# wcy199705/DfFintheWild

Hardware: AMD Instinct MI355X
Metric: focal-stacks/sec (10x3x256x256) (higher is better)
Workload: dtype bf16x3 (split-bf16 MFMA operands hi+lo, fp32 accumulate, fp32-accurate); 1 GPU; DFF_net forward, 10-slice 3x256x256 focal stacks, batch 32 per GPU (BASELINE.json config 3), dense focus_dists, synthetic weights seed 0; batch_per_gpu=32, global_batch=32, slices=10, height=256, width=256, parallelism=single GPU, precision=bf16x3, input=float32 (B,3,N,H,W), the reference's tensor contract

## Files before the change

dffinthewild_amd/csrc/dffw_engine.cpp:

```cpp
#include <algorithm>
#include <cmath>
#include <cstdarg>
#include <cstdio>
#include <cstdlib>
#include <cstring>
#include <functional>
#include <map>
#include <memory>
#include <string>
#include <vector>

#include "dffw_run.h"
#include "dffw_srd_roll.h"
#include "dffw_stem.h"

namespace dffw {

static thread_local std::string g_err;
static thread_local std::string g_last_kernel;
static thread_local std::string g_last_op_kernels;
}
int dffw_fail(int code, const char *fmt, ...) {
    char buf[1024];
    va_list ap;
// ... 1012 lines not shown
}

int dffw_op_efd(int device, int precision, const float *x, int B, int Cin, int N, int H, int W, const float *ws, const float *bns,
                const float *wp, const float *bnp, int pooled_at_hand, float *y, void *hip_stream) {
    g_last_op_kernels.clear();
    if (!x || !ws || !bns || !wp || !bnp || !y) return fail(DFFW_EINVAL, "null argument");
    if (precision < 0 || precision > 2) return fail(DFFW_EINVAL, "unknown precision %d", precision);
    if (Cin != 8 && Cin != 16) return fail(DFFW_EINVAL, "the EFD blocks have 8 or 16 input channels, got %d", Cin);
    if (B < 1 || N < 1 || H < 2 || W < 2 || H % 2 || W % 2) return fail(DFFW_EINVAL, "bad shape (H and W must be even)");
    HIPCHK(hipSetDevice(device));
    const std::string p = Cin == 8 ? "DFF_net.FM_conv1.0" : "DFF_net.FM_conv2.0";
    const int Cout = 2 * Cin;
    Table t;
    t.efd(p, Cin, Cout);
    dffw_engine eng;
    eng.device = device;
    eng.prec = precision;
    const float *const wts[2] = {ws, wp}, *const bnv[2] = {bns, bnp};
    for (int i = 0; i < 2; ++i) {
        const int rc = pack_conv(t.layers[i], precision, wts[i], bnv[i], nullptr, eng.convs[t.layers[i].conv]);
        if (rc) return rc;
    }
    return run_block_op(eng, (hipStream_t)hip_stream, [&](Run &r) {
        Act in = r.act(B, N, H, W, Cin);
        if (r.ok() && !r.dry) r.check(launch_from_ncdhw(precision, x, in.p, B, Cin, N, H, W, r.s), "from_ncdhw");
        Act m;
        if (pooled_at_hand) m = r.pool(in, 0, 2);
        Act out = efd(r, p, in, &m);
        if (r.ok() && !r.dry) r.check(launch_to_ncdhw(precision, out.p, y, B, Cout, N, H / 2, W / 2, r.s), "to_ncdhw");
    });
}

int dffw_op_of_block(int device, int precision, const float *x, int B, int Cin, int N, int H, int W, int Cout, int stride,
                     const float *w0, const float *bn0, const float *w2, const float *bn2, const float *wf, float *y, void *hip_stream) {
    g_last_op_kernels.clear();
    if (!x || !w0 || !bn0 || !w2 || !bn2 || !wf || !y) return fail(DFFW_EINVAL, "null argument");
    if (precision < 0 || precision > 2) return fail(DFFW_EINVAL, "unknown precision %d", precision);
    static const struct { int cin, cout, s; const char *name; } blocks[] = {
        {3, 8, 1, "OF_feature.0"}, {8, 8, 1, "OF_feature.1"}, {8, 16, 2, "OF_feature1.0"},
        {16, 16, 1, "OF_feature1.1"}, {16, 32, 2, "OF_feature2.0"}, {32, 32, 1, "OF_feature2.1"}};
    const char *name = nullptr;
    for (const auto &b : blocks)
        if (b.cin == Cin && b.cout == Cout && b.s == stride) name = b.name;
    if (!name) return fail(DFFW_EINVAL, "no alignment feature block has (Cin, Cout, stride) = (%d, %d, %d)", Cin, Cout, stride);
    if (B < 1 || N < 1 || H < 1 || W < 1 || H % stride || W % stride) return fail(DFFW_EINVAL, "bad shape (H and W must be multiples of the stride)");
    HIPCHK(hipSetDevice(device));
    const std::string p = std::string("optical_flow_aggregation.") + name;
    Table t;
    t.of_block(p, Cin, Cout, stride);
    dffw_engine eng;
    eng.device = device;
    eng.prec = precision;
    for (const LayerDef &L : t.layers) {
        if (L.folded) continue;
        const bool sc = !L.shortcut.empty();
        const float *w = L.conv == p + ".conv.0.0" ? w0 : L.conv == p + ".conv.2.0" ? w2 : wf;
        const float *bn = L.conv == p + ".conv.0.0" ? bn0 : L.conv == p + ".conv.2.0" ? bn2 : nullptr;
        const int rc = pack_conv(L, precision, w, bn, nullptr, eng.convs[L.conv], sc ? wf : nullptr, sc ? Cin : 0);
        if (rc) return rc;
    }
    return run_block_op(eng, (hipStream_t)hip_stream, [&](Run &r) {
        Act out;
        if (Cin == 3) {
            out = of_first_block(r, p, x, B, N, H, W);
        } else {
            Act in = r.act(B, N, H, W, Cin);
            if (r.ok() && !r.dry) r.check(launch_from_ncdhw(precision, x, in.p, B, Cin, N, H, W, r.s), "from_ncdhw");
            out = of_block(r, p, in);
        }
        if (r.ok() && !r.dry) r.check(launch_to_ncdhw(precision, out.p, y, B, Cout, N, H / stride, W / stride, r.s), "to_ncdhw");
    });
}

int dffw_op_regress(int device, const float *score, int B, int N, int h, int w, int H, int W, const float *focus_dists,
                    const int64_t fd_strides[4], float *depth, void *hip_stream) {
    if (!score || !focus_dists || !fd_strides || !depth) return fail(DFFW_EINVAL, "null argument");
    HIPCHK(hipSetDevice(device));
    hipStream_t s = (hipStream_t)hip_stream;
    HIPCHK(launch_regress(score, B, N, h, w, H, W, focus_dists, fd_strides[0], fd_strides[1], fd_strides[2], fd_strides[3], depth, s));
    HIPCHK(hipStreamSynchronize(s));
    return DFFW_OK;
}

int dffw_op_fov_warp(int device, const float *x, int B, int C, int N, int H, int W, const float *alpha, const float *fovs,
                     int alpha_from_sample0, float *out, float *flow, void *hip_stream) {
    if (!x || !alpha || !fovs || !out) return fail(DFFW_EINVAL, "null argument");
    if (B < 1 || C < 1 || N < 1 || H < 1 || W < 1) return fail(DFFW_EINVAL, "bad shape");
    HIPCHK(hipSetDevice(device));
    hipStream_t s = (hipStream_t)hip_stream;
    HIPCHK(launch_fov_warp(x, alpha, fovs, out, flow, B, C, N, H, W, alpha_from_sample0, s));
    HIPCHK(hipStreamSynchronize(s));
    return DFFW_OK;
}

}
```

dffinthewild_amd/csrc/dffw_kernels.hip:

```cpp
#include <cstdio>
#include <cstdlib>

#include "dffw_device.h"
#include "dffw_internal.h"
#include "dffw_persist.h"

namespace dffw {

template <int PREC, int NT, int MT>
__global__ __launch_bounds__(256) void conv_igemm(const ConvArgs a) {
    constexpr int PARTS = Fmt<PREC>::PARTS;
    constexpr bool F16 = (PREC == P_FP16);
    const int lane = threadIdx.x & 63;
    const int wave = threadIdx.x >> 6;
    const int g = lane >> 4, r = lane & 15;
    const int64_t pos0 = ((int64_t)blockIdx.x * 4 + wave) * (MT * 16);
    if (pos0 >= a.M) return;

    const int ps0 = PARTS * a.C0, ps1 = PARTS * a.C1;
    const int64_t samp0 = (int64_t)a.Ni * a.Hi * a.Wi * ps0;
    const int64_t samp1 = (int64_t)a.Ni * a.Hi * a.Wi * ps1;

    int pn[MT], py[MT], px[MT], pbase[MT];
    bool pv[MT];
// ... 1083 lines not shown
                    const float v = hy * (hx * s00[k] + lx * s01[k]) + ly * (hx * s10[k] + lx * s11[k]);
                    const float p = softplus_fast(v) + 1e-6f;
                    den += p;
                    num += f[k] * p;
                }
            }
        }
        depth[i] = num / den;
    }
}

template <int NMAX>
__global__ __launch_bounds__(256) void regress_fused_kernel(const RegressHeads hd, int B, int N, int H, int W, const float *__restrict__ fd, int64_t fsb,
                                                            int64_t fsn, int64_t fsh, int64_t fsw) {
    const unsigned total = (unsigned)B * H * W;
    for (unsigned u = blockIdx.x * blockDim.x + threadIdx.x; u < total; u += gridDim.x * blockDim.x) {
        const unsigned t = u / (unsigned)W;
        const int X = (int)(u - t * (unsigned)W);
        const unsigned bb = t / (unsigned)H;
        const int Y = (int)(t - bb * (unsigned)H);
        const float *fp = fd + bb * fsb + Y * fsh + X * fsw;
        float f[NMAX];
#pragma unroll
        for (int n = 0; n < NMAX; ++n) f[n] = fp[(n < N ? n : N - 1) * fsn];
        for (int head = 0; head < hd.n; ++head) {
            const float *__restrict__ score = hd.score[head];
            const int h = hd.h[head], w = hd.w[head];
            const float *sp = score + (int64_t)bb * N * h * w;
            float num = 0.f, den = 0.f;
            if (h == H && w == W) {
                const int o = Y * w + X;
                float sv[NMAX];
#pragma unroll
                for (int n = 0; n < NMAX; ++n) sv[n] = sp[(int64_t)(n < N ? n : N - 1) * h * w + o];
#pragma unroll
                for (int n = 0; n < NMAX; ++n) {
                    if (n < N) {
                        const float p = softplus_fast(sv[n]) + 1e-6f;
                        den += p;
                        num += f[n] * p;
                    }
                }
            } else {
                const float sch = (float)h / (float)H, scw = (float)w / (float)W;
                float sy = ((float)Y + 0.5f) * sch - 0.5f;
                float sx = ((float)X + 0.5f) * scw - 0.5f;
                sy = sy < 0.f ? 0.f : sy;
                sx = sx < 0.f ? 0.f : sx;
                const int y0 = (int)sy, x0 = (int)sx;
                const int y1 = y0 + (y0 < h - 1 ? 1 : 0), x1 = x0 + (x0 < w - 1 ? 1 : 0);
                const float ly = sy - (float)y0, lx = sx - (float)x0;
                const float hy = 1.f - ly, hx = 1.f - lx;
                const int o00 = y0 * w + x0, o01 = y0 * w + x1, o10 = y1 * w + x0, o11 = y1 * w + x1;
#pragma unroll
                for (int n0 = 0; n0 < NMAX; n0 += 5) {
                    if (n0 < N) {
                        float s00[5], s01[5], s10[5], s11[5];
#pragma unroll
                        for (int k = 0; k < 5; ++k) {
                            const int n = n0 + k < N ? n0 + k : N - 1;
                            const float *pl = sp + (int64_t)n * h * w;
                            s00[k] = pl[o00];
                            s01[k] = pl[o01];
                            s10[k] = pl[o10];
                            s11[k] = pl[o11];
                        }
#pragma unroll
                        for (int k = 0; k < 5; ++k) {
                            if (n0 + k < N) {
                                const float v = hy * (hx * s00[k] + lx * s01[k]) + ly * (hx * s10[k] + lx * s11[k]);
                                const float p = softplus_fast(v) + 1e-6f;
                                den += p;
                                num += f[n0 + k < NMAX ? n0 + k : NMAX - 1] * p;
                            }
                        }
                    }
                }
            }
            hd.depth[head][u] = num / den;
        }
    }
}

hipError_t launch_regress_heads(const RegressHeads &hd, int B, int N, int H, int W, const float *fd, int64_t fsb, int64_t fsn, int64_t fsh,
                                int64_t fsw, hipStream_t s) {
    if (hd.n < 1 || hd.n > 4) return hipErrorInvalidValue;
    const int64_t total = (int64_t)B * H * W;
    if (hd.n > 1 && N <= 16 && total < (1ll << 31) && !hd.nofuse) {
        if (N <= 10) hipLaunchKernelGGL((regress_fused_kernel<10>), dim3(grid_for(total)), dim3(256), 0, s, hd, B, N, H, W, fd, fsb, fsn, fsh, fsw);
        else hipLaunchKernelGGL((regress_fused_kernel<16>), dim3(grid_for(total)), dim3(256), 0, s, hd, B, N, H, W, fd, fsb, fsn, fsh, fsw);
        return hipGetLastError();
    }
    hipLaunchKernelGGL(regress_kernel, dim3(grid_for(total), (unsigned)hd.n), dim3(256), 0, s, hd, B, N, H, W, fd, fsb, fsn, fsh, fsw);
    return hipGetLastError();
}

hipError_t launch_regress(const float *score, int B, int N, int h, int w, int H, int W, const float *fd, int64_t fsb,
                          int64_t fsn, int64_t fsh, int64_t fsw, float *depth, hipStream_t s) {
    RegressHeads hd{};
    hd.n = 1;
    hd.score[0] = score;
    hd.depth[0] = depth;
    hd.h[0] = h;
    hd.w[0] = w;
    return launch_regress_heads(hd, B, N, H, W, fd, fsb, fsn, fsh, fsw, s);
}

__global__ void set_raw_kernel(RawStack rs, RawStack *dst) { *dst = rs; }
hipError_t launch_set_raw(const RawStack &rs, RawStack *dst, hipStream_t s) {
    hipLaunchKernelGGL(set_raw_kernel, dim3(1), dim3(1), 0, s, rs, dst);
    return hipGetLastError();
}

}
```

dffinthewild_amd/engine.py:

```python
import ctypes
import os
import threading
from ctypes import POINTER, byref, c_char_p, c_float, c_int, c_int64, c_void_p

import torch

_HERE = os.path.dirname(os.path.abspath(__file__))
LIB_PATH = os.environ.get("DFFW_LIB_PATH") or os.path.join(_HERE, "libdffw.so")

PRECISIONS = {"bf16x3": 0, "fp16": 1, "bf16": 2}
NET_DEPTH = 0
NET_E2E = 1


class DffwError(RuntimeError):
    pass


class _Tensor(ctypes.Structure):
    _fields_ = [("name", c_char_p), ("data", POINTER(c_float)), ("numel", c_int64)]


class _Tap(ctypes.Structure):
    _fields_ = [("name", c_char_p), ("dst", c_void_p), ("numel", c_int64)]


class _Prof(ctypes.Structure):
    _fields_ = [("kernel", c_char_p), ("layer", c_char_p), ("flops", ctypes.c_double), ("bytes", ctypes.c_double),
                ("ms", c_float)]


class SimParams(ctypes.Structure):
    _fields_ = [("pixel_per_meter", ctypes.c_double), ("min_depth", ctypes.c_double), ("max_depth", ctypes.c_double),
                ("min_focus", ctypes.c_double), ("max_focus", ctypes.c_double), ("num_planes", c_int), ("max_radius", c_int)]


def _load():
    if not os.path.exists(LIB_PATH):
        raise DffwError(
            f"{LIB_PATH} not found: build the HIP extension first "
            "(python -c 'import __graft_entry__ as g; g.build()' or make -C dffinthewild_amd/csrc). "
            "dffinthewild_amd has no CPU fallback.")
    lib = ctypes.CDLL(LIB_PATH)
    lib.dffw_version.restype = c_char_p
    lib.dffw_last_error.restype = c_char_p
    lib.dffw_last_conv_kernel.restype = c_char_p
    lib.dffw_param_count.argtypes = [c_int]
    lib.dffw_param_info.argtypes = [c_int, c_int, POINTER(c_char_p), POINTER(c_int64), POINTER(c_int), POINTER(c_int)]
    lib.dffw_engine_create.argtypes = [c_int, c_int, POINTER(_Tensor), c_int, c_int, POINTER(c_void_p)]
    lib.dffw_engine_destroy.argtypes = [c_void_p]
    lib.dffw_engine_destroy.restype = None
    lib.dffw_engine_precision.argtypes = [c_void_p]
    lib.dffw_workspace_bytes.argtypes = [c_void_p, c_int, c_int, c_int, c_int]
    lib.dffw_workspace_bytes.restype = c_int64
    fwd = [c_void_p, c_void_p, c_void_p, POINTER(c_int64), c_int, c_int, c_int, c_int,
           POINTER(c_void_p), c_void_p, c_int64, c_void_p]
    lib.dffw_forward.argtypes = fwd
    lib.dffw_forward_taps.argtypes = fwd + [POINTER(_Tap), c_int]
    lib.dffw_forward_e2e.argtypes = [c_void_p, c_void_p, c_void_p, POINTER(c_int64), c_void_p, c_int, c_int, c_int, c_int,
                                     POINTER(c_void_p), c_void_p, c_void_p, c_int64, c_void_p, POINTER(_Tap), c_int]
    lib.dffw_forward_raw.argtypes = [c_void_p, c_void_p, c_int, POINTER(c_int64), c_int, c_int, c_void_p, POINTER(c_int64), c_int, c_int, c_int,
                                     c_int, POINTER(c_void_p), c_void_p, c_int64, c_void_p]
    lib.dffw_profile_enable.argtypes = [c_void_p, c_int]
    lib.dffw_profile_collect.argtypes = [c_void_p, POINTER(_Prof), c_int]
    lib.dffw_op_conv3d.argtypes = [c_int, c_int, c_void_p, c_int, c_int, c_int, c_int, c_int, POINTER(c_float), c_int,
                                   POINTER(c_int), POINTER(c_int), POINTER(c_int), POINTER(c_int), c_int,
                                   POINTER(c_float), POINTER(c_float), c_void_p, c_int, c_void_p, c_void_p]
    lib.dffw_op_conv3d_ex.argtypes = [c_int, c_int, c_void_p, c_int, c_int, c_int, c_int, c_int, POINTER(c_float), c_int,
                                      POINTER(c_int), POINTER(c_int), POINTER(c_int), POINTER(c_int), c_int,
                                      POINTER(c_float), POINTER(c_float), c_void_p, c_int, c_void_p, c_void_p, POINTER(c_float), c_void_p, c_void_p]
    lib.dffw_op_pool.argtypes = [c_int, c_int, c_int, c_int, c_void_p, c_int, c_int, c_int, c_int, c_int, c_void_p, c_void_p]
    lib.dffw_op_srd.argtypes = [c_int, c_int, c_void_p, c_int, c_int, c_int, c_int, c_int] + [POINTER(c_float)] * 6 + [c_void_p] * 3
    lib.dffw_op_efd.argtypes = [c_int, c_int, c_void_p, c_int, c_int, c_int, c_int, c_int] + [POINTER(c_float)] * 4 + [c_int, c_void_p, c_void_p]
    lib.dffw_op_of_block.argtypes = [c_int, c_int, c_void_p] + [c_int] * 7 + [POINTER(c_float)] * 5 + [c_void_p] * 2
    lib.dffw_last_op_kernels.restype = c_char_p
    lib.dffw_op_fov_warp.argtypes = [c_int, c_void_p, c_int, c_int, c_int, c_int, c_int, c_void_p, c_void_p, c_int,
                                     c_void_p, c_void_p, c_void_p]
    lib.dffw_op_regress.argtypes = [c_int, c_void_p, c_int, c_int, c_int, c_int, c_int, c_int, c_void_p,
                                    POINTER(c_int64), c_void_p, c_void_p]
    c_u8p = POINTER(ctypes.c_uint8)
    lib.dffw_pack_stack.argtypes = [c_int, c_void_p, c_int, POINTER(c_int64), c_int, c_int, c_int, c_int, c_int, c_int, c_void_p, c_void_p]
    lib.dffw_augment_stack.argtypes = [c_int, c_void_p, c_int, POINTER(c_int64)] + [c_int] * 6 + [c_void_p, c_int] + [c_void_p] * 6 + \
                                      [c_int, c_float, c_float, c_float, c_void_p]
    lib.dffw_unpack_stack.argtypes = [c_int, c_void_p, c_int, c_int, c_int, c_int, c_int, c_int, c_void_p, c_void_p]
    lib.dffw_colorize.argtypes = [c_int, c_void_p, c_int, c_int, c_int, c_int, c_int, c_int, c_float, c_float, c_void_p, c_void_p, c_void_p]
    lib.dffw_jet_lut.argtypes = [c_u8p]
    lib.dffw_metrics_scratch_bytes.argtypes = [c_int]
    lib.dffw_metrics_scratch_bytes.restype = c_int64
    lib.dffw_metrics.argtypes = [c_int, c_void_p, c_int, c_int, c_int, c_void_p, c_void_p, c_void_p, c_int, c_int, c_void_p, c_void_p,
                                 c_int64, c_void_p]
    lib.dffw_comm_unique_id.argtypes = [ctypes.c_char_p]
    lib.dffw_comm_init_rank.argtypes = [c_int, c_int, c_int, ctypes.c_char_p, POINTER(c_void_p)]
    lib.dffw_comm_init_all.argtypes = [c_int, POINTER(c_int), POINTER(c_void_p)]
    lib.dffw_comm_destroy.argtypes = [c_void_p]
    lib.dffw_comm_destroy.restype = None
    lib.dffw_comm_rank.argtypes = [c_void_p]
    lib.dffw_comm_size.argtypes = [c_void_p]
    lib.dffw_allgather.argtypes = [c_void_p, c_void_p, c_void_p, c_int64, c_void_p]
    lib.dffw_probe_peaks.argtypes = [c_int, POINTER(c_float), POINTER(c_float), c_void_p]
    lib.dffw_sim_workspace_bytes.argtypes = [c_int, c_int, c_int, c_int, c_int]
    lib.dffw_sim_workspace_bytes.restype = c_int64
    lib.dffw_sim_render.argtypes = [c_int, SimParams, c_void_p, c_void_p, c_void_p, c_void_p, c_int, c_int, c_int, c_int] + [c_void_p] * 7 + [c_int64, c_void_p]
    lib.dffw_sim_plan_host.argtypes = [POINTER(SimParams), POINTER(ctypes.c_double), ctypes.c_double, ctypes.c_double, c_int,
                                       POINTER(ctypes.c_double), POINTER(c_int), POINTER(ctypes.c_double), POINTER(ctypes.c_double), POINTER(c_int)]
    lib.dffw_sim_disk_rows.argtypes = [c_int, POINTER(c_int)]
    lib.dffw_loss_workspace_bytes.argtypes = [c_int, c_int, c_int, c_int]
    lib.dffw_loss_workspace_bytes.restype = c_int64
    lib.dffw_loss_heads.argtypes = [c_int, c_int, POINTER(c_void_p), POINTER(c_int), POINTER(c_int), c_int, c_int, c_int, c_int, c_void_p, POINTER(c_int64),
                                    c_void_p, c_void_p, c_void_p, POINTER(c_float), c_int, c_float, c_float, POINTER(c_void_p), POINTER(c_void_p),
                                    c_void_p, c_void_p, c_int64, c_void_p]
    lib.dffw_op_conv3d_backward.argtypes = [c_int, c_int, c_void_p, c_int, c_int, c_int, c_int, c_int, POINTER(c_float), c_int,
                                            POINTER(c_int), POINTER(c_int), POINTER(c_int), c_int, c_void_p, c_void_p, c_void_p, c_void_p]
    lib.dffw_conv_wgrad_workspace_bytes.argtypes = [c_int] * 6 + [POINTER(c_int)] * 3 + [c_int]
    lib.dffw_conv_wgrad_workspace_bytes.restype = c_int64
    lib.dffw_conv_wgrad.argtypes = [c_int, c_int, c_void_p, c_int, c_int, c_int, c_int, c_int, c_void_p, c_int,
                                    POINTER(c_int), POINTER(c_int), POINTER(c_int), c_int, c_void_p, c_void_p, c_int64, c_void_p]
    return lib


lib = _load()
COMM_ID_BYTES = 128
RAW_NORM_F64 = 16
AUG_NPARAMS = 8

ABI_SYMBOLS = (
    "dffw_version", "dffw_last_error", "dffw_param_count", "dffw_param_info", "dffw_engine_create",
    "dffw_engine_destroy", "dffw_engine_precision", "dffw_workspace_bytes", "dffw_forward",
    "dffw_forward_taps", "dffw_profile_enable", "dffw_profile_collect", "dffw_op_conv3d", "dffw_op_conv3d_ex", "dffw_op_pool", "dffw_op_regress",
    "dffw_op_fov_warp", "dffw_forward_e2e", "dffw_last_conv_kernel", "dffw_op_srd", "dffw_op_efd", "dffw_last_op_kernels",
    "dffw_op_of_block",
    "dffw_forward_raw", "dffw_pack_stack", "dffw_augment_stack", "dffw_unpack_stack", "dffw_colorize", "dffw_jet_lut", "dffw_metrics_scratch_bytes", "dffw_metrics",
    "dffw_comm_unique_id", "dffw_comm_init_rank", "dffw_comm_init_all", "dffw_comm_destroy", "dffw_comm_rank", "dffw_comm_size",
    "dffw_allgather", "dffw_comm_group_start", "dffw_comm_group_end", "dffw_probe_peaks",
    "dffw_sim_workspace_bytes", "dffw_sim_render", "dffw_sim_plan_host", "dffw_sim_disk_rows",
    "dffw_loss_workspace_bytes", "dffw_loss_heads",
    "dffw_op_conv3d_backward", "dffw_conv_wgrad_workspace_bytes", "dffw_conv_wgrad",
)


def _check(rc, what):
    if rc < 0:
        msg = lib.dffw_last_error().decode("utf-8", "replace")
        if rc == -1:
            raise ValueError(f"{what}: {msg}")
        raise DffwError(f"{what} failed ({rc}): {msg}")
    return rc


def param_table(net=NET_DEPTH):
    n = _check(lib.dffw_param_count(net), "dffw_param_count")
    out = []
    for i in range(n):
        name, shape, ndim, flags = c_char_p(), (c_int64 * 5)(), c_int(), c_int()
        _check(lib.dffw_param_info(net, i, byref(name), shape, byref(ndim), byref(flags)), "dffw_param_info")
        out.append((name.value.decode(), tuple(shape[:ndim.value]), flags.value))
    return out


def _stream_ptr(device):
    return c_void_p(torch.cuda.current_stream(device).cuda_stream)


def _f32(t):
    return ctypes.cast(t.data_ptr(), POINTER(c_float))


class Engine:

    def __init__(self, state_dict, device, precision="bf16x3", net=NET_DEPTH):
        if precision not in PRECISIONS:
            raise ValueError(f"precision must be one of {sorted(PRECISIONS)}, got {precision!r}")
        self.device = torch.device(device)
        if self.device.type != "cuda":
            raise DffwError("the HIP engine needs a GPU device (no CPU fallback)")
        self.index = self.device.index if self.device.index is not None else torch.cuda.current_device()
        self.precision = precision
        keep, arr = [], (_Tensor * len(state_dict))()
        i = 0
        for key, t in state_dict.items():
            if not torch.is_floating_point(t):
                continue
            h = t.detach().to("cpu", torch.float32).contiguous()
            keep.append(h)
            arr[i] = _Tensor(key.encode(), _f32(h), h.numel())
            i += 1
        self._h = c_void_p()
        _check(lib.dffw_engine_create(self.index, net, arr, i, PRECISIONS[precision], byref(self._h)), "dffw_engine_create")
        self._ws = {}
        self._ws_stream = None
        self._lock = threading.Lock()

    def __copy__(self):
        raise TypeError("dffinthewild_amd.engine.Engine cannot be copied: build a new one from the state dict")

    def __deepcopy__(self, memo):
        raise TypeError("dffinthewild_amd.engine.Engine cannot be copied: build a new one from the state dict")

    def __reduce__(self):
        raise TypeError("dffinthewild_amd.engine.Engine cannot be pickled: save the model's state_dict instead")

    def __del__(self, _destroy=lib.dffw_engine_destroy):
        h = getattr(self, "_h", None)
        if h:
            _destroy(h)
            self._h = None

    def profile(self, on=True):
        _check(lib.dffw_profile_enable(self._h, int(on)), "dffw_profile_enable")

    def profile_collect(self):
        n = _check(lib.dffw_profile_collect(self._h, None, 0), "dffw_profile_collect")
# ... 185 lines not shown
def probe_peaks(device=0):
    m, h = c_float(), c_float()
    with torch.cuda.device(device):
        _check(lib.dffw_probe_peaks(device, byref(m), byref(h), _stream_ptr(device)), "dffw_probe_peaks")
    return m.value, h.value


def last_conv_kernel():
    return lib.dffw_last_conv_kernel().decode()


def _host_f32(t):
    return t.detach().to("cpu", torch.float32).contiguous()


def _bn_host(bn):
    return torch.cat([_host_f32(t).reshape(-1) for t in bn]).contiguous()


def op_srd(x, w0, bn0, w2, bn2, w3, w1, *, pooled=False, precision="bf16x3"):
    B, C, N, H, W = x.shape
    x = x.contiguous()
    y = torch.empty_like(x)
    pl = torch.empty((B, C, N, H // 2, W // 2), dtype=torch.float32, device=x.device) if pooled else None
    host = [_host_f32(w0), _bn_host(bn0), _host_f32(w2), _bn_host(bn2), _host_f32(w3), _host_f32(w1)]
    dev = x.device.index if x.device.index is not None else torch.cuda.current_device()
    with torch.cuda.device(dev):
        _check(lib.dffw_op_srd(dev, PRECISIONS[precision], c_void_p(x.data_ptr()), B, C, N, H, W, *[_f32(t) for t in host],
                               c_void_p(y.data_ptr()), c_void_p(pl.data_ptr()) if pooled else None, _stream_ptr(dev)), "dffw_op_srd")
    return (y, pl) if pooled else y


def op_efd(x, ws, bns, wp, bnp, *, pooled_at_hand=True, precision="bf16x3"):
    B, C, N, H, W = x.shape
    x = x.contiguous()
    y = torch.empty((B, 2 * C, N, H // 2, W // 2), dtype=torch.float32, device=x.device)
    host = [_host_f32(ws), _bn_host(bns), _host_f32(wp), _bn_host(bnp)]
    dev = x.device.index if x.device.index is not None else torch.cuda.current_device()
    with torch.cuda.device(dev):
        _check(lib.dffw_op_efd(dev, PRECISIONS[precision], c_void_p(x.data_ptr()), B, C, N, H, W, *[_f32(t) for t in host],
                               int(bool(pooled_at_hand)), c_void_p(y.data_ptr()), _stream_ptr(dev)), "dffw_op_efd")
    return y


def op_of_block(x, w0, bn0, w2, bn2, wf, *, stride=1, precision="bf16x3"):
    B, C, N, H, W = x.shape
    Cout = w0.shape[0]
    x = x.contiguous()
    y = torch.empty((B, Cout, N, H // stride, W // stride), dtype=torch.float32, device=x.device)
    host = [_host_f32(w0), _bn_host(bn0), _host_f32(w2), _bn_host(bn2), _host_f32(wf)]
    dev = x.device.index if x.device.index is not None else torch.cuda.current_device()
    with torch.cuda.device(dev):
        _check(lib.dffw_op_of_block(dev, PRECISIONS[precision], c_void_p(x.data_ptr()), B, C, N, H, W, Cout, stride,
                                    *[_f32(t) for t in host], c_void_p(y.data_ptr()), _stream_ptr(dev)), "dffw_op_of_block")
    return y


def op_kernels():
    s = lib.dffw_last_op_kernels().decode()
    return s.split(";") if s else []


def op_pool(x, k, mode="max", precision="bf16x3"):
    B, C, N, H, W = x.shape
    y = torch.empty((B, C, N, H // k, W // k), dtype=torch.float32, device=x.device)
    x = x.contiguous()
    dev = x.device.index if x.device.index is not None else torch.cuda.current_device()
    with torch.cuda.device(dev):
        _check(lib.dffw_op_pool(dev, PRECISIONS[precision], 0 if mode == "max" else 1, k, c_void_p(x.data_ptr()),
                                B, C, N, H, W, c_void_p(y.data_ptr()), _stream_ptr(dev)), "dffw_op_pool")
    return y


def op_regress(score, focus_dists, H, W):
    B, N, h, w = score.shape
    score = score.contiguous()
    fd = focus_dists.expand(B, N, H, W)
    depth = torch.empty((B, H, W), dtype=torch.float32, device=score.device)
    dev = score.device.index if score.device.index is not None else torch.cuda.current_device()
    with torch.cuda.device(dev):
        _check(lib.dffw_op_regress(dev, c_void_p(score.data_ptr()), B, N, h, w, H, W, c_void_p(fd.data_ptr()),
                                   (c_int64 * 4)(*fd.stride()), c_void_p(depth.data_ptr()), _stream_ptr(dev)),
               "dffw_op_regress")
    return depth


def loss_workspace_bytes(B, N, H, W):
    return int(lib.dffw_loss_workspace_bytes(B, N, H, W))


def op_loss_heads(scores, focus_dists, gt, mask, conf=None, weights=(0.3, 0.5, 0.7, 1.0), depth_range=None, *, preds=True, grads=True,
                  workspace=None):
    n = len(scores)
    B, H, W = gt.shape
    N = scores[0].shape[1]
    dev = scores[0].device.index if scores[0].device.index is not None else torch.cuda.current_device()
    device = scores[0].device
    scores = [s.contiguous() for s in scores]
    for s in scores:
        if s.dtype != torch.float32 or s.dim() != 4 or s.shape[0] != B or s.shape[1] != N:
            raise ValueError(f"score volumes must be float32 (B,N,h,w) with B={B}, N={N}; got {s.dtype} {tuple(s.shape)}")
    gt, mask = gt.contiguous(), mask.contiguous()
    if gt.dtype != torch.float32 or mask.dtype != torch.uint8 or tuple(mask.shape) != (B, H, W):
        raise ValueError("gt must be float32 (B,H,W) and mask uint8 of the same shape")
    if conf is not None:
        conf = conf.contiguous()
        if conf.dtype != torch.float32 or tuple(conf.shape) != (B, H, W):
            raise ValueError("conf must be float32 (B,H,W)")
    if len(weights) < n:
        raise ValueError(f"{n} heads but {len(weights)} weights")
    fd = focus_dists.expand(B, N, H, W)
    pred = [torch.empty((B, H, W), dtype=torch.float32, device=device) for _ in range(n)] if preds else None
    grad = [torch.empty_like(s) for s in scores] if grads else None
    losses = torch.empty(n + 1, dtype=torch.float64, device=device)
    need = loss_workspace_bytes(B, N, H, W)
    ws = workspace if workspace is not None else torch.empty(max(need, 8), dtype=torch.uint8, device=device)
    ptrs = lambda ts: (c_void_p * 4)(*[t.data_ptr() for t in ts]) if ts is not None else None
    lo, hi = (0.0, 1.0) if depth_range is None else (float(depth_range[0]), float(depth_range[1]))
    with torch.cuda.device(dev):
        _check(lib.dffw_loss_heads(dev, n, ptrs(scores), (c_int * 4)(*[s.shape[2] for s in scores]), (c_int * 4)(*[s.shape[3] for s in scores]),
                                   B, N, H, W, c_void_p(fd.data_ptr()), (c_int64 * 4)(*fd.stride()), c_void_p(gt.data_ptr()), c_void_p(mask.data_ptr()),
                                   c_void_p(conf.data_ptr()) if conf is not None else None, (c_float * 4)(*[float(x) for x in weights[:n]]),
                                   0 if depth_range is None else 1, lo, hi, ptrs(pred), ptrs(grad), c_void_p(losses.data_ptr()),
                                   c_void_p(ws.data_ptr()), ws.numel(), _stream_ptr(dev)), "dffw_loss_heads")
    return losses, pred, grad


def op_fov_warp(x, alpha, fovs, compat_batch_alpha0=False):
    B, C, N, H, W = x.shape
    x = x.contiguous()
    a = alpha.reshape(B, 3, N).contiguous().float()
    f = fovs.reshape(B, N).contiguous().float()
    out = torch.empty_like(x)
    flow = torch.empty((B, 2, N, H, W), dtype=torch.float32, device=x.device)
    dev = x.device.index if x.device.index is not None else torch.cuda.current_device()
    with torch.cuda.device(dev):
        _check(lib.dffw_op_fov_warp(dev, c_void_p(x.data_ptr()), B, C, N, H, W, c_void_p(a.data_ptr()), c_void_p(f.data_ptr()),
                                    int(compat_batch_alpha0), c_void_p(out.data_ptr()), c_void_p(flow.data_ptr()),
                                    _stream_ptr(dev)), "dffw_op_fov_warp")
    return out, flow


SIM_LDS_RADIUS = 32
SIM_NSCALARS = 12
SIM_SCALARS = ("fd", "fd_px", "lens_to_sensor", "fov", "coc_scale", "f_px", "lens_dia", "scene_min", "scene_max", "min_afov",
               "max_afov", "origin_max_afov")


def sim_params(pixel_per_meter, depth_range, focus_range, num_planes, max_radius=-1):
    return SimParams(float(pixel_per_meter), float(depth_range[0]), float(depth_range[1]), float(focus_range[0]),
                     float(focus_range[1]), int(num_planes), int(max_radius))


def sim_plan_host(params, cam, dmin, dmax, N):
    import numpy as np
    P = params.num_planes
    sc = np.zeros((N, SIM_NSCALARS), np.float64)
    coc = np.zeros((N, P), np.int32)
    lo = np.zeros((N, P), np.float64)
    hi = np.zeros((N, P), np.float64)
    nl = np.zeros(N, np.int32)
    dp = POINTER(ctypes.c_double)
    camv = (ctypes.c_double * 4)(*[float(v) for v in cam])
    _check(lib.dffw_sim_plan_host(byref(params), camv, float(dmin), float(dmax), N, sc.ctypes.data_as(dp),
                                  coc.ctypes.data_as(POINTER(c_int)), lo.ctypes.data_as(dp), hi.ctypes.data_as(dp),
                                  nl.ctypes.data_as(POINTER(c_int))), "dffw_sim_plan_host")
# ... 44 lines not shown
```

include/dffw.h:

```cpp
#ifndef DFFW_H
#define DFFW_H

#include <stdint.h>

#ifdef __cplusplus
extern "C" {
#endif

#define DFFW_OK 0
#define DFFW_EINVAL (-1)
#define DFFW_EHIP (-2)
#define DFFW_ENOMEM (-3)
#define DFFW_EMISSING (-4)

#define DFFW_PREC_BF16X3 0
#define DFFW_PREC_FP16 1
#define DFFW_PREC_BF16 2

#define DFFW_NET_DEPTH 0
#define DFFW_NET_E2E 1
#define DFFW_E2E_SLICES 10

typedef struct dffw_engine dffw_engine;

typedef struct dffw_tensor {
    const char *name;
    const float *data;
    int64_t numel;
} dffw_tensor;

typedef struct dffw_tap {
    const char *name;
    float *dst;
    int64_t numel;
} dffw_tap;

const char *dffw_version(void);
const char *dffw_last_error(void);
const char *dffw_last_conv_kernel(void);

int dffw_param_count(int net);
int dffw_param_info(int net, int index, const char **name, int64_t shape[5], int *ndim, int *flags);

int dffw_engine_create(int device, int net, const dffw_tensor *tensors, int n_tensors,
                       int precision, dffw_engine **out);
void dffw_engine_destroy(dffw_engine *e);
int dffw_engine_precision(const dffw_engine *e);

int64_t dffw_workspace_bytes(const dffw_engine *e, int B, int N, int H, int W);

int dffw_forward(dffw_engine *e, const float *FS, const float *focus_dists,
                 const int64_t fd_strides[4], int B, int N, int H, int W, float *const out[4],
                 void *workspace, int64_t workspace_bytes, void *hip_stream);

int dffw_forward_taps(dffw_engine *e, const float *FS, const float *focus_dists,
                      const int64_t fd_strides[4], int B, int N, int H, int W, float *const out[4],
                      void *workspace, int64_t workspace_bytes, void *hip_stream,
                      const dffw_tap *taps, int n_taps);

int dffw_forward_e2e(dffw_engine *e, const float *FS, const float *focus_dists,
                     const int64_t fd_strides[4], const float *fovs, int B, int N, int H, int W,
                     float *const out[4], float *aligned, void *workspace, int64_t workspace_bytes,
                     void *hip_stream, const dffw_tap *taps, int n_taps);

typedef struct dffw_prof_entry {
    const char *kernel;
    const char *layer;
    double flops;
    double bytes;
    float ms;
} dffw_prof_entry;
int dffw_profile_enable(dffw_engine *e, int on);
int dffw_profile_collect(dffw_engine *e, dffw_prof_entry *out, int capacity);


int dffw_op_conv3d(int device, int precision, const float *x, int B, int Cin, int N, int H, int W,
                   const float *weight, int Cout, const int kernel[3], const int stride[3],
                   const int pad[3], const int dilation[3], int transposed, const float *bn,
                   const float *conv_bias, const float *residual, int relu, float *y,
                   void *hip_stream);

int dffw_op_conv3d_ex(int device, int precision, const float *x, int B, int Cin, int N, int H, int W,
                      const float *weight, int Cout, const int kernel[3], const int stride[3],
                      const int pad[3], const int dilation[3], int transposed, const float *bn,
                      const float *conv_bias, const float *residual, int relu, float *y, float *y_pre,
                      const float *cls_weight, float *cls_score, void *hip_stream);

int dffw_op_pool(int device, int precision, int mode, int k, const float *x, int B, int C, int N,
                 int H, int W, float *y, void *hip_stream);

int dffw_op_srd(int device, int precision, const float *x, int B, int C, int N, int H, int W,
                const float *w0, const float *bn0, const float *w2, const float *bn2, const float *w3,
                const float *w1, float *y, float *pooled, void *hip_stream);

int dffw_op_efd(int device, int precision, const float *x, int B, int Cin, int N, int H, int W,
                const float *ws, const float *bns, const float *wp, const float *bnp, int pooled_at_hand,
                float *y, void *hip_stream);

int dffw_op_of_block(int device, int precision, const float *x, int B, int Cin, int N, int H, int W, int Cout, int stride,
                     const float *w0, const float *bn0, const float *w2, const float *bn2, const float *wf, float *y,
                     void *hip_stream);

const char *dffw_last_op_kernels(void);

int dffw_op_regress(int device, const float *score, int B, int N, int h, int w, int H, int W,
                    const float *focus_dists, const int64_t fd_strides[4], float *depth,
                    void *hip_stream);

int dffw_op_fov_warp(int device, const float *x, int B, int C, int N, int H, int W, const float *alpha,
                     const float *fovs, int alpha_from_sample0, float *out, float *flow, void *hip_stream);

#define DFFW_RAW_U8 0
#define DFFW_RAW_F32 1
#define DFFW_RAW_NORM_F64 16
int dffw_pack_stack(int device, const void *raw, int dtype, const int64_t strides[5], int B, int N, int h, int w,
                    int Hp, int Wp, float *FS, void *hip_stream);

#define DFFW_AUG_NPARAMS 8
enum { DFFW_AUG_Y0, DFFW_AUG_X0, DFFW_AUG_CONTRAST, DFFW_AUG_BRIGHTNESS, DFFW_AUG_GAMMA, DFFW_AUG_FLIP_X, DFFW_AUG_FLIP_Y, DFFW_AUG_ANGLE };
int dffw_augment_stack(int device, const void *raw, int dtype, const int64_t strides[5], int B, int N, int H, int W, int h, int w,
                       const double *params, int transposed, float *FS, const float *gt, const float *conf, float *gt_out,
                       uint8_t *mask_out, float *conf_out, int use_range, float lo, float hi, float sentinel, void *hip_stream);

int dffw_forward_raw(dffw_engine *e, const void *raw, int dtype, const int64_t raw_strides[5], int h, int w,
                     const float *focus_dists, const int64_t fd_strides[4], int B, int N, int H, int W,
                     float *const out[4], void *workspace, int64_t workspace_bytes, void *hip_stream);

#define DFFW_RANGE_FIXED 0
#define DFFW_RANGE_MINMAX 1
int dffw_colorize(int device, const float *depth, int B, int H, int W, int h, int w, int mode, float lo, float hi,
                  float *range, uint8_t *rgb, void *hip_stream);
int dffw_jet_lut(uint8_t *lut768);

int dffw_unpack_stack(int device, const float *warp, int B, int N, int H, int W, int h, int w, uint8_t *images, void *hip_stream);

#define DFFW_N_METRICS 12
int64_t dffw_metrics_scratch_bytes(int B);
int dffw_metrics(int device, const float *est, int B, int H, int W, const float *gt, const uint8_t *mask,
                 const float *conf, int h, int w, double *out, void *scratch, int64_t scratch_bytes, void *hip_stream);

int64_t dffw_loss_workspace_bytes(int B, int N, int H, int W);
int dffw_loss_heads(int device, int n_heads, const float *const score[4], const int h[4], const int w[4],
                    int B, int N, int H, int W, const float *focus_dists, const int64_t fd_strides[4],
                    const float *gt, const uint8_t *mask, const float *conf, const float weights[4],
                    int use_range, float lo, float hi, float *const pred[4], float *const grad[4],
                    double *losses, void *workspace, int64_t workspace_bytes, void *hip_stream);

int dffw_op_conv3d_backward(int device, int precision, const float *x, int B, int Cin, int N, int H, int W, const float *weight, int Cout,
                            const int kernel[3], const int stride[3], const int pad[3], int transposed, const float *grad_y, float *grad_x,
                            float *grad_w, void *hip_stream);
int64_t dffw_conv_wgrad_workspace_bytes(int B, int Cin, int N, int H, int W, int Cout, const int kernel[3], const int stride[3],
                                        const int pad[3], int transposed);
int dffw_conv_wgrad(int device, int precision, const void *x, int B, int Cin, int N, int H, int W, const void *grad_y, int Cout,
                    const int kernel[3], const int stride[3], const int pad[3], int transposed, float *grad_w, void *workspace,
                    int64_t workspace_bytes, void *hip_stream);

typedef struct dffw_sim_params {
    double pixel_per_meter;
    double min_depth, max_depth;
    double min_focus, max_focus;
    int num_planes;
    int max_radius;
} dffw_sim_params;
#define DFFW_SIM_LDS_RADIUS 32
#define DFFW_SIM_DISCARD 1
#define DFFW_SIM_NSCALARS 12
enum { DFFW_SIM_FD, DFFW_SIM_FD_PX, DFFW_SIM_LENS_TO_SENSOR, DFFW_SIM_FOV, DFFW_SIM_COC_SCALE, DFFW_SIM_F_PX, DFFW_SIM_LENS_DIA,
       DFFW_SIM_SCENE_MIN, DFFW_SIM_SCENE_MAX, DFFW_SIM_MIN_AFOV, DFFW_SIM_MAX_AFOV, DFFW_SIM_ORIGIN_MAX_AFOV };

int64_t dffw_sim_workspace_bytes(int B, int N, int H, int W, int num_planes);

int dffw_sim_render(int device, dffw_sim_params params, const double *cams, const float *image, const double *depth,
                    const double *shifts, int B, int N, int H, int W, uint8_t *images, double *defocus, float *depth_out,
                    int32_t *status, double *slices, float *warped_tap, void *workspace, int64_t ws_bytes, void *hip_stream);

int dffw_sim_plan_host(const dffw_sim_params *params, const double cam[4], double dmin, double dmax, int N, double *scalars,
                       int *coc, double *lo, double *hi, int *nlayers);

int dffw_sim_disk_rows(int r, int *halfwidths);

int dffw_probe_peaks(int device, float *mfma_tflops, float *hbm_gbs, void *hip_stream);

#define DFFW_COMM_ID_BYTES 128
typedef struct dffw_comm dffw_comm;
int dffw_comm_unique_id(char id[DFFW_COMM_ID_BYTES]);
int dffw_comm_init_rank(int device, int nranks, int rank, const char id[DFFW_COMM_ID_BYTES], dffw_comm **out);
int dffw_comm_init_all(int ndev, const int *devices, dffw_comm **out );
void dffw_comm_destroy(dffw_comm *c);
int dffw_comm_rank(const dffw_comm *c);
int dffw_comm_size(const dffw_comm *c);
// ... 9 lines not shown
```

Baseline: 4086 stacks/s.

## Add tiled vectorized fused multi-head regress kernel with shared-memory score taps

```diff
diff --git a/dffinthewild_amd/csrc/dffw_engine.cpp b/dffinthewild_amd/csrc/dffw_engine.cpp
--- a/dffinthewild_amd/csrc/dffw_engine.cpp
+++ b/dffinthewild_amd/csrc/dffw_engine.cpp
@@ -1118,6 +1118,29 @@
     return DFFW_OK;
 }
 
+int dffw_op_regress_heads(int device, int n_heads, const float *const score[4], const int h[4], const int w[4], int B, int N, int H, int W,
+                          const float *focus_dists, const int64_t fd_strides[4], float *const depth[4], void *hip_stream) {
+    if (!score || !h || !w || !focus_dists || !fd_strides || !depth) return fail(DFFW_EINVAL, "null argument");
+    if (n_heads < 1 || n_heads > 4) return fail(DFFW_EINVAL, "n_heads must be 1..4");
+    if (B < 1 || N < 1 || H < 1 || W < 1) return fail(DFFW_EINVAL, "bad shape");
+    RegressHeads hd{};
+    hd.n = n_heads;
+    for (int k = 0; k < n_heads; ++k) {
+        if (!score[k] || !depth[k]) return fail(DFFW_EINVAL, "null argument");
+        if (h[k] < 1 || w[k] < 1) return fail(DFFW_EINVAL, "bad shape");
+        hd.score[k] = score[k];
+        hd.depth[k] = depth[k];
+        hd.h[k] = h[k];
+        hd.w[k] = w[k];
+    }
+    hd.nofuse = Switches::read().on(SW_NO_REGRESS_FUSED) ? 1 : 0;
+    HIPCHK(hipSetDevice(device));
+    hipStream_t s = (hipStream_t)hip_stream;
+    HIPCHK(launch_regress_heads(hd, B, N, H, W, focus_dists, fd_strides[0], fd_strides[1], fd_strides[2], fd_strides[3], s));
+    HIPCHK(hipStreamSynchronize(s));
+    return DFFW_OK;
+}
+
 int dffw_op_fov_warp(int device, const float *x, int B, int C, int N, int H, int W, const float *alpha, const float *fovs,
                      int alpha_from_sample0, float *out, float *flow, void *hip_stream) {
     if (!x || !alpha || !fovs || !out) return fail(DFFW_EINVAL, "null argument");
diff --git a/dffinthewild_amd/csrc/dffw_kernels.hip b/dffinthewild_amd/csrc/dffw_kernels.hip
--- a/dffinthewild_amd/csrc/dffw_kernels.hip
+++ b/dffinthewild_amd/csrc/dffw_kernels.hip
@@ -1189,11 +1189,195 @@
     }
 }
 
+__device__ __forceinline__ float mul_rn(float a, float b) {
+#pragma clang fp contract(off)
+    return a * b;
+}
+__device__ __forceinline__ float add_rn(float a, float b) {
+#pragma clang fp contract(off)
+    return a + b;
+}
+__device__ __forceinline__ float bilinear_pinned(bool first2, float hy, float ly, float hx, float lx, float s00, float s01, float s10, float s11) {
+    const float row0 = first2 ? __builtin_fmaf(lx, s01, mul_rn(hx, s00)) : __builtin_fmaf(hx, s00, mul_rn(lx, s01));
+    const float row1 = first2 ? __builtin_fmaf(hx, s10, mul_rn(lx, s11)) : __builtin_fmaf(lx, s11, mul_rn(hx, s10));
+    return add_rn(mul_rn(hy, row0), mul_rn(ly, row1));
+}
+constexpr int RV_TW = 64, RV_TH = 16;
+constexpr int RV_SLICE = (RV_TH / 2 + 2) * ((RV_TW / 2 + 2) | 1);
+enum { FD_SCALAR = 0, FD_VEC4 = 1, FD_BCAST = 2 };
+
+template <int NMAX, int FDM>
+__global__ __launch_bounds__(256) void regress_fused_vec_kernel(const RegressHeads hd, int N, int H, int W, const float *__restrict__ fd, int64_t fsb,
+                                                                int64_t fsn, int64_t fsh, int64_t fsw) {
+    static_assert(NMAX % 2 == 0, "slices are consumed in pairs");
+    __shared__ float tap[NMAX * RV_SLICE];
+    constexpr int FW = FDM == FD_BCAST ? 1 : 4;
+    const int tid = threadIdx.x;
+    const int X0 = blockIdx.x * RV_TW, Y0 = blockIdx.y * RV_TH;
+    const unsigned bb = blockIdx.z;
+    const int X = X0 + (tid & 15) * 4, Y = Y0 + (tid >> 4);
+    const bool live = X < W && Y < H;
+    float f[NMAX][FW];
+    if (FDM == FD_BCAST) {
+#pragma unroll
+        for (int n = 0; n < NMAX; ++n) f[n][0] = fd[bb * fsb + (n < N ? n : N - 1) * fsn];
+    } else if (live) {
+        const float *fp = fd + bb * fsb + Y * fsh + X * fsw;
+#pragma unroll
+        for (int n = 0; n < NMAX; ++n) {
+            const float *q = fp + (n < N ? n : N - 1) * fsn;
+            if (FDM == FD_VEC4) {
+                const float4 t = *reinterpret_cast<const float4 *>(q);
+                f[n][0] = t.x; f[n][FW > 1 ? 1 : 0] = t.y; f[n][FW > 1 ? 2 : 0] = t.z; f[n][FW > 1 ? 3 : 0] = t.w;
+            } else {
+#pragma unroll
+                for (int k = 0; k < FW; ++k) f[n][k] = q[k * fsw];
+            }
+        }
+    } else {
+#pragma unroll
+        for (int n = 0; n < NMAX; ++n)
+#pragma unroll
+            for (int k = 0; k < FW; ++k) f[n][k] = 0.f;
+    }
+    const size_t opix = ((size_t)bb * H + Y) * W + X;
+    for (int head = 0; head < hd.n; ++head) {
+        const int h = hd.h[head], w = hd.w[head];
+        const size_t plane = (size_t)h * w;
+        const float *sp = hd.score[head] + (size_t)bb * N * plane;
+        float num[4] = {0.f, 0.f, 0.f, 0.f}, den[4] = {0.f, 0.f, 0.f, 0.f};
+        if (h == H && w == W) {
+            if (live) {
+                const unsigned o = (unsigned)(Y * w + X);
+                float4 sv[NMAX];
+#pragma unroll
+                for (int n = 0; n < NMAX; ++n) sv[n] = *reinterpret_cast<const float4 *>(sp + (size_t)(n < N ? n : N - 1) * plane + o);
+#pragma unroll
+                for (int n = 0; n < NMAX; ++n) {
+                    if (n < N) {
+                        const float v[4] = {sv[n].x, sv[n].y, sv[n].z, sv[n].w};
+#pragma unroll
+                        for (int k = 0; k < 4; ++k) {
+                            const float p = softplus_fast(v[k]) + 1e-6f;
+                            den[k] += p;
+                            num[k] = add_rn(num[k], mul_rn(f[n][k < FW ? k : 0], p));
+                        }
+                    }
+                }
+                *reinterpret_cast<float4 *>(hd.depth[head] + opix) = make_float4(num[0] / den[0], num[1] / den[1], num[2] / den[2], num[3] / den[3]);
+            }
+            continue;
+        }
+        const int s = H / h;
+        const int fw = RV_TW / s + 2, fh = RV_TH / s + 2, rs = fw | 1;
+        const int xb = X0 / s - 1, yb = Y0 / s - 1;
+        __syncthreads();
+        for (int e = tid; e < fw * fh; e += 256) {
+            const int r = e / fw, c = e - r * fw;
+            int gy = yb + r, gx = xb + c;
+            gy = gy < 0 ? 0 : (gy > h - 1 ? h - 1 : gy);
+            gx = gx < 0 ? 0 : (gx > w - 1 ? w - 1 : gx);
+            const unsigned o = (unsigned)(gy * w + gx);
+            float t[NMAX];
+#pragma unroll
+            for (int n = 0; n < NMAX; ++n) t[n] = sp[(size_t)(n < N ? n : N - 1) * plane + o];
+#pragma unroll
+            for (int n = 0; n < NMAX; ++n) tap[n * RV_SLICE + r * rs + c] = t[n];
+        }
+        __syncthreads();
+        if (live) {
+            const float sch = (float)h / (float)H, scw = (float)w / (float)W;
+            float sy = ((float)Y + 0.5f) * sch - 0.5f;
+            sy = sy < 0.f ? 0.f : sy;
+            const int y0 = (int)sy;
+            const int y1 = y0 + (y0 < h - 1 ? 1 : 0);
+            const float ly = sy - (float)y0;
+            const float hy = 1.f - ly;
+            const int r0 = (y0 - yb) * rs - xb, r1 = (y1 - yb) * rs - xb;
+            int a00[4], a01[4], a10[4], a11[4];
+            float lx[4], hx[4];
+#pragma unroll
+            for (int k = 0; k < 4; ++k) {
+                float sx = ((float)(X + k) + 0.5f) * scw - 0.5f;
+                sx = sx < 0.f ? 0.f : sx;
+                const int x0 = (int)sx;
+                const int x1 = x0 + (x0 < w - 1 ? 1 : 0);
+                lx[k] = sx - (float)x0;
+                hx[k] = 1.f - lx[k];
+                a00[k] = r0 + x0; a01[k] = r0 + x1; a10[k] = r1 + x0; a11[k] = r1 + x1;
+            }
+#pragma unroll
+            for (int n0 = 0; n0 < NMAX; n0 += 2) {
+                if (n0 < N) {
+                    float s00[2][4], s01[2][4], s10[2][4], s11[2][4];
+#pragma unroll
+                    for (int j = 0; j < 2; ++j) {
+                        const float *t = tap + (n0 + j) * RV_SLICE;
+#pragma unroll
+                        for (int k = 0; k < 4; ++k) {
+                            s00[j][k] = t[a00[k]];
+                            s01[j][k] = t[a01[k]];
+                            s10[j][k] = t[a10[k]];
+                            s11[j][k] = t[a11[k]];
+                        }
+                    }
+#pragma unroll
+                    for (int j = 0; j < 2; ++j) {
+                        if (n0 + j < N) {
+#pragma unroll
+                            for (int k = 0; k < 4; ++k) {
+                                const float v = bilinear_pinned((n0 + j) % 5 < 2, hy, ly, hx[k], lx[k], s00[j][k], s01[j][k], s10[j][k], s11[j][k]);
+                                const float p = softplus_fast(v) + 1e-6f;
+                                den[k] += p;
+                                num[k] = add_rn(num[k], mul_rn(f[n0 + j][k < FW ? k : 0], p));
+                            }
+                        }
+                    }
+                }
+            }
+            *reinterpret_cast<float4 *>(hd.depth[head] + opix) = make_float4(num[0] / den[0], num[1] / den[1], num[2] / den[2], num[3] / den[3]);
+        }
+    }
+}
+
+static inline bool aligned16(const void *p) { return (reinterpret_cast<uintptr_t>(p) & 15) == 0; }
+
+static bool regress_vec_takes(const RegressHeads &hd, int B, int H, int W) {
+    if (W % 4 || B > 65535) return false;
+    for (int k = 0; k < hd.n; ++k) {
+        if (!aligned16(hd.depth[k])) return false;
+        if (hd.h[k] == H && hd.w[k] == W) {
+            if (!aligned16(hd.score[k])) return false;
+            continue;
+        }
+        const int s = hd.h[k] > 0 ? H / hd.h[k] : 0;
+        if ((s != 2 && s != 4 && s != 8) || hd.h[k] * s != H || hd.w[k] * s != W) return false;
+    }
+    return true;
+}
+
+template <int NMAX>
+static void launch_regress_vec(const RegressHeads &hd, int B, int N, int H, int W, const float *fd, int64_t fsb, int64_t fsn, int64_t fsh, int64_t fsw,
+                               hipStream_t s) {
+    const dim3 grid((W + RV_TW - 1) / RV_TW, (H + RV_TH - 1) / RV_TH, B);
+    if (fsh == 0 && fsw == 0)
+        hipLaunchKernelGGL((regress_fused_vec_kernel<NMAX, FD_BCAST>), grid, dim3(256), 0, s, hd, N, H, W, fd, fsb, fsn, fsh, fsw);
+    else if (fsw == 1 && aligned16(fd) && fsh % 4 == 0 && fsn % 4 == 0 && fsb % 4 == 0)
+        hipLaunchKernelGGL((regress_fused_vec_kernel<NMAX, FD_VEC4>), grid, dim3(256), 0, s, hd, N, H, W, fd, fsb, fsn, fsh, fsw);
+    else
+        hipLaunchKernelGGL((regress_fused_vec_kernel<NMAX, FD_SCALAR>), grid, dim3(256), 0, s, hd, N, H, W, fd, fsb, fsn, fsh, fsw);
+}
+
 hipError_t launch_regress_heads(const RegressHeads &hd, int B, int N, int H, int W, const float *fd, int64_t fsb, int64_t fsn, int64_t fsh,
                                 int64_t fsw, hipStream_t s) {
     if (hd.n < 1 || hd.n > 4) return hipErrorInvalidValue;
     const int64_t total = (int64_t)B * H * W;
     if (hd.n > 1 && N <= 16 && total < (1ll << 31) && !hd.nofuse) {
+        if (regress_vec_takes(hd, B, H, W)) {
+            if (N <= 10) launch_regress_vec<10>(hd, B, N, H, W, fd, fsb, fsn, fsh, fsw, s);
+            else launch_regress_vec<16>(hd, B, N, H, W, fd, fsb, fsn, fsh, fsw, s);
+            return hipGetLastError();
+        }
         if (N <= 10) hipLaunchKernelGGL((regress_fused_kernel<10>), dim3(grid_for(total)), dim3(256), 0, s, hd, B, N, H, W, fd, fsb, fsn, fsh, fsw);
         else hipLaunchKernelGGL((regress_fused_kernel<16>), dim3(grid_for(total)), dim3(256), 0, s, hd, B, N, H, W, fd, fsb, fsn, fsh, fsw);
         return hipGetLastError();
diff --git a/dffinthewild_amd/engine.py b/dffinthewild_amd/engine.py
--- a/dffinthewild_amd/engine.py
+++ b/dffinthewild_amd/engine.py
@@ -78,6 +78,8 @@
                                      c_void_p, c_void_p, c_void_p]
     lib.dffw_op_regress.argtypes = [c_int, c_void_p, c_int, c_int, c_int, c_int, c_int, c_int, c_void_p,
                                     POINTER(c_int64), c_void_p, c_void_p]
+    lib.dffw_op_regress_heads.argtypes = [c_int, c_int, POINTER(c_void_p), POINTER(c_int), POINTER(c_int), c_int, c_int, c_int, c_int, c_void_p,
+                                          POINTER(c_int64), POINTER(c_void_p), c_void_p]
     c_u8p = POINTER(ctypes.c_uint8)
     lib.dffw_pack_stack.argtypes = [c_int, c_void_p, c_int, POINTER(c_int64), c_int, c_int, c_int, c_int, c_int, c_int, c_void_p, c_void_p]
     lib.dffw_augment_stack.argtypes = [c_int, c_void_p, c_int, POINTER(c_int64)] + [c_int] * 6 + [c_void_p, c_int] + [c_void_p] * 6 + \
@@ -127,6 +129,7 @@
     "dffw_version", "dffw_last_error", "dffw_param_count", "dffw_param_info", "dffw_engine_create",
     "dffw_engine_destroy", "dffw_engine_precision", "dffw_workspace_bytes", "dffw_forward",
     "dffw_forward_taps", "dffw_profile_enable", "dffw_profile_collect", "dffw_op_conv3d", "dffw_op_conv3d_ex", "dffw_op_pool", "dffw_op_regress",
+    "dffw_op_regress_heads",
     "dffw_op_fov_warp", "dffw_forward_e2e", "dffw_last_conv_kernel", "dffw_op_srd", "dffw_op_efd", "dffw_last_op_kernels",
     "dffw_op_of_block",
     "dffw_forward_raw", "dffw_pack_stack", "dffw_augment_stack", "dffw_unpack_stack", "dffw_colorize", "dffw_jet_lut", "dffw_metrics_scratch_bytes", "dffw_metrics",
@@ -478,6 +481,30 @@
         _check(lib.dffw_op_regress(dev, c_void_p(score.data_ptr()), B, N, h, w, H, W, c_void_p(fd.data_ptr()),
                                    (c_int64 * 4)(*fd.stride()), c_void_p(depth.data_ptr()), _stream_ptr(dev)),
                "dffw_op_regress")
+    return depth
+
+
+def op_regress_heads(scores, focus_dists, H, W, out=None):
+    n = len(scores)
+    B, N = scores[0].shape[:2]
+    scores = [s.contiguous() for s in scores]
+    for s in scores:
+        if s.dtype != torch.float32 or s.dim() != 4 or s.shape[0] != B or s.shape[1] != N:
+            raise ValueError(f"score volumes must be float32 (B,N,h,w) with B={B}, N={N}; got {s.dtype} {tuple(s.shape)}")
+    device = scores[0].device
+    fd = focus_dists.expand(B, N, H, W)
+    depth = out if out is not None else [torch.empty((B, H, W), dtype=torch.float32, device=device) for _ in range(n)]
+    for d in depth:
+        if d.dtype != torch.float32 or tuple(d.shape) != (B, H, W) or not d.is_contiguous():
+            raise ValueError("out must be contiguous float32 (B,H,W) tensors")
+    if len(depth) != n:
+        raise ValueError(f"{n} heads but {len(depth)} outputs")
+    dev = device.index if device.index is not None else torch.cuda.current_device()
+    ptrs = lambda ts: (c_void_p * 4)(*[t.data_ptr() for t in ts])
+    with torch.cuda.device(dev):
+        _check(lib.dffw_op_regress_heads(dev, n, ptrs(scores), (c_int * 4)(*[s.shape[2] for s in scores]), (c_int * 4)(*[s.shape[3] for s in scores]),
+                                         B, N, H, W, c_void_p(fd.data_ptr()), (c_int64 * 4)(*fd.stride()), ptrs(depth), _stream_ptr(dev)),
+               "dffw_op_regress_heads")
     return depth
 
 
diff --git a/include/dffw.h b/include/dffw.h
--- a/include/dffw.h
+++ b/include/dffw.h
@@ -106,6 +106,10 @@
 int dffw_op_regress(int device, const float *score, int B, int N, int h, int w, int H, int W,
                     const float *focus_dists, const int64_t fd_strides[4], float *depth,
                     void *hip_stream);
+
+int dffw_op_regress_heads(int device, int n_heads, const float *const score[4], const int h[4], const int w[4],
+                          int B, int N, int H, int W, const float *focus_dists, const int64_t fd_strides[4],
+                          float *const depth[4], void *hip_stream);
 
 int dffw_op_fov_warp(int device, const float *x, int B, int C, int N, int H, int W, const float *alpha,
                      const float *fovs, int alpha_from_sample0, float *out, float *flow, void *hip_stream);
```

After: 4081 stacks/s. Within noise of the previous version (-0.1%).
